# joyecnu/STTODE

Measured on AMD Instinct MI355X. Metric: predicted-trajectories/sec (20-sample best-of-K), higher is better.
Workload: dtype f32

## Files before the change

sttode_amd/csrc/chain32.hip:

```cpp
#include "chain.hpp"
#include "latency_bodies.hpp"
#include "frontend_body.hpp"
#include "api_util.hpp"
#include "../../include/sttode_hip.h"
#include <cstdlib>
#include <cstddef>

#ifdef C32_DIAG_TRACE
__shared__ long long g_tr_ph[4];
#define C32_TRACE_BEGIN() long long _tr_t0 = 0, _tr_c0 = 0; if (threadIdx.x == 0 && A.dbg) { _tr_t0 = __builtin_amdgcn_s_memrealtime(); _tr_c0 = __builtin_amdgcn_s_memtime(); }
#define C32_TRACE_END(kind) do { if (threadIdx.x == 0 && A.dbg) { \
        const long long _t1 = __builtin_amdgcn_s_memrealtime(); unsigned _hw, _xcc; \
        asm volatile("s_getreg_b32 %0, hwreg(HW_REG_HW_ID)" : "=s"(_hw)); asm volatile("s_getreg_b32 %0, hwreg(HW_REG_XCC_ID)" : "=s"(_xcc)); \
        const unsigned long long _r = atomicAdd((unsigned long long*)A.dbg, 1ull); if ((long long)_r >= A.dbg[1]) break;  \
        long long* _p = A.dbg + 8 + _r * 12; _p[0] = A.trace_tag; _p[1] = blockIdx.x; _p[2] = (kind); _p[3] = _tr_t0; _p[4] = _t1; _p[5] = _hw; _p[6] = _xcc; \
        _p[8] = g_tr_ph[0]; _p[9] = g_tr_ph[1]; _p[10] = g_tr_ph[2]; _p[7] = __builtin_amdgcn_s_memtime() - _tr_c0; _p[11] = g_tr_ph[3]; } } while (0)
#define C32_TRACE_PHASE(i) do { if (threadIdx.x == 0) g_tr_ph[i] = __builtin_amdgcn_s_memrealtime(); } while (0)
#else
#define C32_TRACE_PHASE(i) do { } while (0)
#define C32_TRACE_BEGIN() do { } while (0)
#define C32_TRACE_END(kind) do { } while (0)
#endif

#include "role_body.hpp"
// ... 443 lines not shown
            }
            const f32x4* tc = st.cur() + (i % 3) * C32_TILE_B3;
            const f32x4* tn = (i % 3 < 2) ? tc + C32_TILE_B3 : nullptr;
            if (i > 0 && i < KT1) {
                STT_FENCE();
                split3(Bh[i - 1], Bt);
            }
            f32x16& acc = i < KT1 ? h1 : acc2[i < KT1 ? 0 : i - KT1];
            if (PRE) tile_mma_b3(acc, fr[i & 1], Bt, fr[(i + 1) & 1], tn);
            else tile_mma_b3n(acc, tc, Bt);
            if (i == KT1 - 1) {
                h1 = relu16(h1);
                split3(h1, Bt);
            }
        }
        st.end();
    }
}
template <int NO, class ST>
__device__ __forceinline__ void mlp_l3_b3(ST& st, f32x16 (&acc2)[8], const float* __restrict__ b2, const float* __restrict__ b3,
                                          f32x16 (&out)[NO], int h) {
#pragma unroll
    for (int o = 0; o < NO; ++o) out[o] = ldrows(b3 + 32 * o, h);
    Frag6 fr[2];
    B3 Bt;
#pragma unroll
    for (int i = 0; i < 8 * NO; ++i) {
        if (i % NO == 0) {
            STT_FENCE();
            const f32x16 b = ldrows(b2 + 32 * (i / NO), h);
            const f32x16 a = relu16(acc2[i / NO] + b);
            split3(a, Bt);
        }
        if (i % 3 == 0) {
            if (i > 0) st.end();
            ldfrag6(fr[i & 1], st.cur());
            st.begin();
        }
        const f32x4* tn = (i % 3 < 2 && i + 1 < 8 * NO) ? st.cur() + (i % 3 + 1) * C32_TILE_B3 : nullptr;
        tile_mma_b3(out[i % NO], fr[i & 1], Bt, fr[(i + 1) & 1], tn);
    }
    st.end();
}

__device__ __forceinline__ f32x16 b3_to_f32(const B3& b) {
    f32x16 r;
#pragma unroll
    for (int kb = 0; kb < 2; ++kb) {
        const u32x4v H = __builtin_bit_cast(u32x4v, b.p[0][kb]), M = __builtin_bit_cast(u32x4v, b.p[1][kb]), L = __builtin_bit_cast(u32x4v, b.p[2][kb]);
#pragma unroll
        for (int q = 0; q < 4; ++q) {
            r[8 * kb + 2 * q] = (bf_lo(H[q]) + bf_lo(M[q])) + bf_lo(L[q]);
            r[8 * kb + 2 * q + 1] = (bf_hi(H[q]) + bf_hi(M[q])) + bf_hi(L[q]);
        }
    }
    return r;
}
template <class ST>
__device__ __forceinline__ void gru32_steps_b3(ST& st, const float* gb, const float* cb, const f32x16& d, f32x16 (&hs)[3], int Tp, int h) {
    B3 dB, hB[3];
    split3(d, dB);
#pragma unroll
    for (int j = 0; j < 3; ++j) split3(hs[j], hB[j]);
    constexpr int T = C32_TILE_B3;
#pragma unroll 1
    for (int t = 0; t < Tp; ++t) {
        B3 eB;
        {
            f32x16 e = ldrows(cb, h);
            st.begin();
            tile_mma_b3n(e, st.cur(), dB);
            e = relu16(e);
            st.end();
            split3(e, eB);
        }
        f32x16 hn[3];
#pragma unroll
        for (int j = 0; j < 3; ++j) {
            STT_FENCE();
            f32x16 ar = ldrows(gb + 0 * 96 + 32 * j, h);
            st.begin();
            tile_mma_b3n(ar, st.cur(), eB);
            tile_mma_b3n(ar, st.cur() + T, hB[0]);
            tile_mma_b3n(ar, st.cur() + 2 * T, hB[1]);
            st.end(); st.begin();
            tile_mma_b3n(ar, st.cur(), hB[2]);
#pragma unroll
            for (int r = 0; r < 16; ++r) ar[r] = C32_SIG(ar[r]);
            STT_FENCE();
            f32x16 az = ldrows(gb + 1 * 96 + 32 * j, h);
            tile_mma_b3n(az, st.cur() + T, eB);
            tile_mma_b3n(az, st.cur() + 2 * T, hB[0]);
            st.end(); st.begin();
            tile_mma_b3n(az, st.cur(), hB[1]);
            tile_mma_b3n(az, st.cur() + T, hB[2]);
#pragma unroll
            for (int r = 0; r < 16; ++r) az[r] = C32_SIG(az[r]);
            STT_FENCE();
            f32x16 an = ldrows(gb + 3 * 96 + 32 * j, h);
            tile_mma_b3n(an, st.cur() + 2 * T, hB[0]);
            st.end(); st.begin();
            tile_mma_b3n(an, st.cur(), hB[1]);
            tile_mma_b3n(an, st.cur() + T, hB[2]);
            {
                const f32x16 bi = ldrows(gb + 2 * 96 + 32 * j, h);
#pragma unroll
                for (int r = 0; r < 16; ++r) an[r] = fmaf(ar[r], an[r], bi[r]);
            }
            STT_FENCE();
            tile_mma_b3n(an, st.cur() + 2 * T, eB);
            st.end();
            const f32x16 hp = b3_to_f32(hB[j]);
#pragma unroll
            for (int r = 0; r < 16; ++r) {
                const float ng = C32_TANH(an[r]);
                hn[j][r] = fmaf(az[r], hp[r] - ng, ng);
            }
        }
#pragma unroll
        for (int j = 0; j < 3; ++j) {
            hs[j] = hn[j];
            split3(hn[j], hB[j]);
        }
    }
}

template <bool ZS, class ST>
__device__ __forceinline__ f32x16 gru32_conv(ST& st, const float* cb, const f32x16& d, int t, int Tp, int h, bool pre) {
    f32x16 e = ldrows(cb, h);
    Frag fa, fb;
    if (ZS) {
        const int k0 = 2 * t - 2, k1 = 2 * t + 3;
        const int g0 = (k0 > 0 ? k0 : 0) >> 3, g1 = (k1 < 2 * Tp - 1 ? k1 : 2 * Tp - 1) >> 3;
        const f32x4* tc = st.cur();
#pragma unroll
        for (int g = 0; g < 4; ++g)
            if (g >= g0 && g <= g1) fa.a[g] = tc[g * 64];
        st.begin(3);
#pragma unroll
        for (int g = 0; g < 4; ++g)
            if (g >= g0 && g <= g1)
#pragma unroll
                for (int r = 0; r < 4; ++r) e = __builtin_amdgcn_mfma_f32_32x32x2f32(fa.a[g][r], d[4 * g + r], e, 0, 0, 0);
        __builtin_amdgcn_sched_barrier(0);
        if (pre) st.take_prefetched();
        else st.fetch();
    } else {
        ldfrag(fa, st.cur());
        st.begin(3);
        tile_mma2f(st, e, fa, d, fb, nullptr, pre ? 0 : 1);
        if (pre) st.take_prefetched();
    }
    e = relu16(e);
    st.end();
    return e;
}

template <bool ZS, class ST>
__device__ __forceinline__ void gru32_steps(ST& st, const float* gb, const float* cb, const f32x16& d, f32x16 (&hs)[3], int Tp, int h) {
    if (ZS) {
        const f32x16 e = gru32_conv<ZS>(st, cb, d, 0, Tp, h, false);
        Frag fa, fb;
#pragma unroll
        for (int j = 0; j < 3; ++j) {
            STT_FENCE();
            f32x16 ar = ldrows(gb + 0 * 96 + 32 * j, h);
            ldfrag(fa, st.cur()); st.begin(3);
            tile_mma2f(st, ar, fa, e, fb, nullptr);
            st.end(); ldfrag(fa, st.cur() + 1 * C32_TILE); st.begin(3);
#pragma unroll
            for (int r = 0; r < 16; ++r) ar[r] = C32_SIG(ar[r]);
            STT_FENCE();
            f32x16 az = ldrows(gb + 1 * 96 + 32 * j, h);
            tile_mma2f(st, az, fa, e, fb, nullptr, 2);
            st.end(); st.begin(3);
            st.take_prefetched();
#pragma unroll
            for (int r = 0; r < 16; ++r) az[r] = C32_SIG(az[r]);
            STT_FENCE();
            f32x16 an = ldrows(gb + 3 * 96 + 32 * j, h);
            {
                const f32x16 bi = ldrows(gb + 2 * 96 + 32 * j, h);
#pragma unroll
                for (int r = 0; r < 16; ++r) an[r] = fmaf(ar[r], an[r], bi[r]);
            }
            st.end(); ldfrag(fa, st.cur() + 2 * C32_TILE);
            if (j < 2) st.begin(3); else st.begin();
            STT_FENCE();
            tile_mma2f(st, an, fa, e, fb, nullptr, (j == 2 && 1 < Tp) ? 2 : 1);
            st.end();
#pragma unroll
            for (int r = 0; r < 16; ++r) {
                const float ng = C32_TANH(an[r]);
                hs[j][r] = fmaf(az[r], 0.f - ng, ng);
            }
        }
    }
#pragma unroll 1
    for (int t = ZS ? 1 : 0; t < Tp; ++t) {
        const f32x16 e = gru32_conv<ZS>(st, cb, d, t, Tp, h, ZS);
        Frag fa, fb;
        f32x16 hn[3];
#pragma unroll
        for (int j = 0; j < 3; ++j) {
            STT_FENCE();
            f32x16 ar = ldrows(gb + 0 * 96 + 32 * j, h);
            ldfrag(fa, st.cur()); st.begin(3);
            tile_mma2f(st, ar, fa, e, fb, st.cur() + 1 * C32_TILE);
            tile_mma2(ar, fb, hs[0], fa, st.cur() + 2 * C32_TILE);
            tile_mma2(ar, fa, hs[1], fb, nullptr);
            st.end(); ldfrag(fa, st.cur()); st.begin(3);
            tile_mma2f(st, ar, fa, hs[2], fb, st.cur() + 1 * C32_TILE);
#pragma unroll
            for (int r = 0; r < 16; ++r) ar[r] = C32_SIG(ar[r]);
            STT_FENCE();
            f32x16 az = ldrows(gb + 1 * 96 + 32 * j, h);
            tile_mma2(az, fb, e, fa, st.cur() + 2 * C32_TILE);
            tile_mma2(az, fa, hs[0], fb, nullptr);
            st.end(); ldfrag(fa, st.cur()); st.begin(3);
            tile_mma2f(st, az, fa, hs[1], fb, st.cur() + 1 * C32_TILE);
            tile_mma2(az, fb, hs[2], fa, st.cur() + 2 * C32_TILE);
#pragma unroll
            for (int r = 0; r < 16; ++r) az[r] = C32_SIG(az[r]);
            STT_FENCE();
            f32x16 an = ldrows(gb + 3 * 96 + 32 * j, h);
            tile_mma2(an, fa, hs[0], fb, nullptr);
            st.end(); ldfrag(fa, st.cur());
            if (j < 2) st.begin(3); else st.begin();
            tile_mma2f(st, an, fa, hs[1], fb, st.cur() + 1 * C32_TILE, (ZS && j == 2 && t + 1 < Tp) ? 2 : 1);
            tile_mma2(an, fb, hs[2], fa, st.cur() + 2 * C32_TILE);
            {
                const f32x16 bi = ldrows(gb + 2 * 96 + 32 * j, h);
#pragma unroll
                for (int r = 0; r < 16; ++r) an[r] = fmaf(ar[r], an[r], bi[r]);
            }
            STT_FENCE();
            tile_mma2(an, fa, e, fb, nullptr);
            st.end();
#pragma unroll
            for (int r = 0; r < 16; ++r) {
                const float ng = C32_TANH(an[r]);
                hn[j][r] = fmaf(az[r], hs[j][r] - ng, ng);
            }
        }
#pragma unroll
        for (int j = 0; j < 3; ++j) hs[j] = hn[j];
    }

}

#include "role32.hpp"

__device__ __forceinline__ int opaque(int v) { asm volatile("" : "+v"(v)); return v; }

#ifdef C32_DIAG_STAMPS
#define C32_STAMP(k) do { if (threadIdx.x == 0 && A.dbg && gi < 4) { A.dbg[((size_t)blockIdx.x * 4 + gi) * 16 + 2 * (k)] = __builtin_amdgcn_s_memtime(); \
                                                                    A.dbg[((size_t)blockIdx.x * 4 + gi) * 16 + 2 * (k) + 1] = __builtin_amdgcn_s_memrealtime(); } } while (0)
#else
#define C32_STAMP(k) do { } while (0)
#endif


__host__ __device__ __forceinline__ int xcd_group(int b, int G) {
    const int x = b & 7, i = b >> 3, q = G >> 3, r = G & 7;
    return x * q + (x < r ? x : r) + i;
}

template <int NY, int FUSE, bool B3M, bool ZS>
__global__ __launch_bounds__(256, 2) void traj_chain_kernel(ChainArgs A) {
    constexpr bool kDynCount = !B3M && ((NY == 1 && FUSE == 2 && !ZS) || (NY == 2 && FUSE == 1 && ZS));
    typedef ChainStreamT<B3M ? C32_BUF_B3 : C32_CMAX * C32_TILE, B3M, kDynCount> Stream;
    extern __shared__ __attribute__((aligned(16))) char smem[];
    f32x4* ring = reinterpret_cast<f32x4*>(smem);
    f32x4* slots = ring + 2 * Stream::kBuf;
    f32x4* zslots = slots + 4 * C32_SLOT;
    float* cst = reinterpret_cast<float*>(zslots + 4 * C32_SLOT);
    int* sq = reinterpret_cast<int*>(cst + C32Const<NY>::total);
    typedef C32Const<NY> CO;

    const int lane = threadIdx.x & 63, c = lane & 31, h = lane >> 5;
    const int wave = __builtin_amdgcn_readfirstlane(threadIdx.x >> 6);
    const f32x4* slot = slots + wave * C32_SLOT;
    const f32x4* zslot = zslots + wave * C32_SLOT;
    const unsigned slot_addr = __builtin_amdgcn_readfirstlane(lds_addr(slot));
    const unsigned zslot_addr = __builtin_amdgcn_readfirstlane(lds_addr(zslot));
    const int ngroups = (A.ncols + 127) >> 7;

    C32_TRACE_BEGIN();
    if (FUSE == 2 && (int)blockIdx.x < A.R32.nwg) {
        role32_body<ZS>(*(KRole32Args*)((const __attribute__((address_space(4))) char*)__builtin_amdgcn_kernarg_segment_ptr() + offsetof(ChainArgs, R32)),
                    blockIdx.x, smem);
        C32_TRACE_END(1);
        return;
    }
    int fb = FUSE == 0 ? (int)blockIdx.x : (int)blockIdx.x - (FUSE == 2 ? A.R32.nwg : A.R.ntiles);
    if (FUSE && A.xcd_map && fb >= 0) fb = xcd_group(fb, ngroups);
    if (FUSE == 1 && fb < 0) {
        agent_role(A.R, (A.ncols + A.K - 1) / A.K, A.Tp, A.ldx, A.xpad, A.R.ntiles + fb, smem);
        C32_TRACE_END(1);
        return;
    }
    for (int i = threadIdx.x; i < CO::total; i += blockDim.x) cst[i] = A.consts[i];
    if (threadIdx.x == 0) sq[0] = FUSE == 2 ? fb : (FUSE == 0 && A.persistent) ? atomicAdd(A.counter, 1) : FUSE ? fb : (int)blockIdx.x;
    if (FUSE == 1) {
        const int g0 = fb;
        const int c_lo = g0 * 128, c_hi = (c_lo + 127 < A.ncols ? c_lo + 127 : A.ncols - 1);
        const int t_lo = (c_lo / A.K) >> 4, t_hi = (c_hi / A.K) >> 4;
        if (wave == 0) {
            const bool ok = wait_tiles(A.R.flags, t_lo, t_hi, A.R.flags + A.R.ntiles, lane, A.R.tmo_host);
            if (!ok && lane == 0) sq[0] = -1;
        }
    }
    __syncthreads();
    C32_TRACE_PHASE(3);
    int g = sq[0];
    if (FUSE == 1 && g < 0) {
        for (int i = threadIdx.x; i < 128 * A.Tf2; i += blockDim.x) {
            const size_t o = (size_t)fb * 128 * A.Tf2 + i;
            if (o < (size_t)A.ncols * A.Tf2) A.pred[o] = __builtin_nanf("");
        }
        return;
    }
    if (g >= ngroups) return;
    Stream st;
    st.init(A.pool, A.prog, A.prog_len, ring);

    auto col_of = [&](int gg) { int col = gg * 128 + wave * 32 + c; return col < A.ncols ? col : A.ncols - 1; };
    {
        const int c0 = col_of(g);
        gather_rows(A.A0x, row_off(c0 / A.K, 512, h), slot_addr);
        gather_rows(A.z, row_off(c0, 32, h), zslot_addr);
    }
    asm volatile("s_waitcnt vmcnt(0)" ::: "memory");
    __syncthreads();

    int gi = 0;
    (void)gi;
    while (true) {
        C32_STAMP(0);
        const int col = g * 128 + wave * 32 + c;
        int colc = col < A.ncols ? col : A.ncols - 1;
        int agent = colc / A.K;
        const bool live = col < A.ncols;
        __syncthreads();
        if (threadIdx.x == 0)
            sq[1] = (FUSE == 2 && A.persistent && ngroups > A.nworkers) ? A.nworkers + atomicAdd(A.counter, 1)
                    : (FUSE == 0 && A.persistent) ? atomicAdd(A.counter, 1) : ngroups;

        f32x16 acc2[8];
        f32x16 d;
        {
            agent = opaque(agent);
            f32x16 xo[1];
            const unsigned ao = row_off(agent, 512, h);
            if (B3M) {
                mlp_l12_b3<0, true>(st, slot, zslot, nullptr, A.A0x, ao, A.A0y, ao, acc2, lane);
                mlp_l3_b3<1>(st, acc2, cst + CO::b2x, cst + CO::b3x, xo, h);
            } else {
                mlp_l12<0>(st, slot, zslot, nullptr, A.A0x, ao, A.A0y, ao, acc2, lane);
                mlp_l3<1, 3>(st, acc2, cst + CO::b2x, cst + CO::b3x, xo, h);
            }
            agent = opaque(agent);
            const float* xp = A.xpad + (size_t)agent * A.ldx;
#pragma unroll
            for (int a = 0; a < 4; ++a) {
                f32x4 v = splat4(0.f);
                if (8 * a + 4 * h < A.ldx) v = ld4(xp + 8 * a + 4 * h);
#pragma unroll
                for (int b = 0; b < 4; ++b) d[4 * a + b] = v[b] - xo[0][4 * a + b];
            }
        }
        STT_FENCE();
        C32_STAMP(1);
        {
            agent = opaque(agent);
            f32x16 yo[NY];
            const unsigned ao = row_off(agent, 512, h);
            if (B3M) {
                mlp_l12_b3<0, true>(st, slot, zslot, nullptr, A.A0y, ao, A.A1y, ao, acc2, lane);
                mlp_l3_b3<NY>(st, acc2, cst + CO::b2y, cst + CO::b3y, yo, h);
            } else {
                mlp_l12<0>(st, slot, zslot, nullptr, A.A0y, ao, A.A1y, ao, acc2, lane);
                mlp_l3<NY, 1>(st, acc2, cst + CO::b2y, cst + CO::b3y, yo, h);
            }
            if (live) {
                float* prow = A.park + (size_t)opaque(col) * A.Tf2;
#pragma unroll
                for (int o = 0; o < NY; ++o)
#pragma unroll
                    for (int a = 0; a < 4; ++a) {
                        const int row0 = 32 * o + 8 * a + 4 * h;
                        float* p = prow + row0;
                        if (row0 + 3 < A.Tf2 && (A.Tf2 & 3) == 0) {
                            f32x4 v = {yo[o][4 * a], yo[o][4 * a + 1], yo[o][4 * a + 2], yo[o][4 * a + 3]};
                            st4(p, v);
                        } else {
#pragma unroll
                            for (int b = 0; b < 4; ++b)
                                if (row0 + b < A.Tf2) p[b] = yo[o][4 * a + b];
                        }
                    }
            }
        }
        STT_FENCE();
        C32_STAMP(2);
        f32x16 hs[3];
        {
#pragma unroll
            for (int j = 0; j < 3; ++j) hs[j] = splat16(0.f);
            if (B3M) gru32_steps_b3(st, cst + CO::gb, cst + CO::cb, d, hs, A.Tp, h);
            else gru32_steps<ZS>(st, cst + CO::gb, cst + CO::cb, d, hs, A.Tp, h);
        }
        STT_FENCE();
        C32_STAMP(3);
        const int gnext = sq[1];
        {
            agent = opaque(agent);
            const int cnx = col_of(gnext < ngroups ? gnext : g);
            const unsigned ao = row_off(agent, 512, h), an = row_off(cnx / A.K, 512, h);
            if (B3M) mlp_l12_b3<3, false>(st, slot, zslot, hs, A.A1y, ao, A.A0x, an, acc2, lane);
            else mlp_l12<3>(st, slot, zslot, hs, A.A1y, ao, A.A0x, an, acc2, lane);
            gather_rows(A.z, row_off(opaque(cnx), 32, h), zslot_addr);
            f32x16 yo[NY];
            if (B3M) mlp_l3_b3<NY>(st, acc2, cst + CO::b2m, cst + CO::b3m, yo, h);
            else mlp_l3<NY, 3>(st, acc2, cst + CO::b2m, cst + CO::b3m, yo, h);
            {
                agent = opaque(agent);
                const float cx = A.cur[2 * agent], cy = A.cur[2 * agent + 1];
                const float ox = A.orig[2 * agent], oy = A.orig[2 * agent + 1];
                const bool vec = (A.Tf2 & 3) == 0;
                const float* yrow = A.park + (size_t)opaque(colc) * A.Tf2;
                float* prow = A.pred + (size_t)opaque(col) * A.Tf2;
                const float* grow = FUSE == 2 && A.m_gt ? A.m_gt + (size_t)agent * A.Tf2 : nullptr;
                float dd[NY][4][2];
#pragma unroll
                for (int o = 0; o < NY; ++o)
#pragma unroll
                    for (int a = 0; a < 4; ++a) {
                        const int row0 = 32 * o + 8 * a + 4 * h;
                        const bool whole = vec && row0 + 3 < A.Tf2;
                        f32x4 y0 = splat4(0.f);
                        if (whole) y0 = ld4(yrow + row0);
                        else {
#pragma unroll
                            for (int b = 0; b < 4; ++b)
                                if (row0 + b < A.Tf2) y0[b] = yrow[row0 + b];
                        }
                        f32x4 v;
                        v[0] = ((y0[0] + yo[o][4 * a + 0]) + cx) + ox;
                        v[1] = ((y0[1] + yo[o][4 * a + 1]) + cy) + oy;
                        v[2] = ((y0[2] + yo[o][4 * a + 2]) + cx) + ox;
                        v[3] = ((y0[3] + yo[o][4 * a + 3]) + cy) + oy;
                        if (live) {
                            if (whole) st4(prow + row0, v);
                            else {
#pragma unroll
                                for (int b = 0; b < 4; ++b)
                                    if (row0 + b < A.Tf2) prow[row0 + b] = v[b];
                            }
                        }
                        dd[o][a][0] = dd[o][a][1] = 0.f;
                        if (FUSE == 2 && grow) {
                            if (row0 < A.Tf2) { const float2 g = *reinterpret_cast<const float2*>(grow + row0); dd[o][a][0] = bok_dist(v[0], v[1], g.x, g.y, A.m_scale); }
                            if (row0 + 2 < A.Tf2) { const float2 g = *reinterpret_cast<const float2*>(grow + row0 + 2); dd[o][a][1] = bok_dist(v[2], v[3], g.x, g.y, A.m_scale); }
                        }
                    }
                if (FUSE == 2 && grow) {
                    const int Tf = A.Tf2 >> 1;
                    float acc = 0.f, fdl = -1.f;
#pragma unroll
                    for (int o = 0; o < NY; ++o)
#pragma unroll
                        for (int a = 0; a < 4; ++a) {
                            const int t0 = (32 * o + 8 * a + 4 * h) >> 1;
                            float mine = acc;
                            if (h == 0) { if (t0 < Tf) mine += dd[o][a][0]; if (t0 + 1 < Tf) mine += dd[o][a][1]; }
                            float mine1 = __shfl(mine, c, 64);
                            if (h == 1) { if (t0 < Tf) mine1 += dd[o][a][0]; if (t0 + 1 < Tf) mine1 += dd[o][a][1]; }
                            acc = __shfl(mine1, c + 32, 64);
                            if (t0 == Tf - 1) fdl = dd[o][a][0];
                            if (t0 + 1 == Tf - 1) fdl = dd[o][a][1];
                        }
                    fdl = fmaxf(fdl, __shfl_xor(fdl, 32, 64));
                    const float adev = acc / (float)Tf;
                    if (live && h == 0) {
                        atomicMin(reinterpret_cast<unsigned*>(A.m_ade) + agent, __float_as_uint(adev));
                        atomicMin(reinterpret_cast<unsigned*>(A.m_fde) + agent, __float_as_uint(fdl));
                    }
                }
            }
        }
        C32_STAMP(4);
#ifdef C32_DIAG_STAMPS
        if (threadIdx.x == 0 && A.dbg && gi < 4) {
            long long* o = A.dbg + ((size_t)blockIdx.x * 4 + gi) * 16 + 10;
            o[0] = st.gap_cyc; o[1] = st.gap_n; o[2] = st.gap_cal;
        }
        st.gap_cyc = 0; st.gap_n = 0;
#endif
        ++gi;
        g = gnext;
        if (g >= ngroups) break;
    }
    C32_TRACE_END(0);
}

struct Gru32Args {
    const float* xin; int ldx;
    const f32x4* pool; const int2* prog; int prog_len;
    const float* consts;
    float* state;
    int ncols, Tp;
};
template <bool ZS>
__global__ __launch_bounds__(256, 2) void gru32_kernel(Gru32Args A) {
    extern __shared__ __attribute__((aligned(16))) char smem[];
    f32x4* ring = reinterpret_cast<f32x4*>(smem);
    float* cst = reinterpret_cast<float*>(ring + C32_RING);
    const int lane = threadIdx.x & 63, c = lane & 31, h = lane >> 5;
    const int wave = __builtin_amdgcn_readfirstlane(threadIdx.x >> 6);
    for (int i = threadIdx.x; i < 416; i += blockDim.x) cst[i] = A.consts[i];
    __syncthreads();
    ChainStream st;
    st.init(A.pool, A.prog, A.prog_len, ring);
    const int col = blockIdx.x * 128 + wave * 32 + c;
    const int colc = col < A.ncols ? col : A.ncols - 1;
    f32x16 d;
    {
        const float* xp = A.xin + (size_t)colc * A.ldx;
#pragma unroll
        for (int a = 0; a < 4; ++a) {
            f32x4 v = splat4(0.f);
            if (8 * a + 4 * h < A.ldx) v = ld4(xp + 8 * a + 4 * h);
#pragma unroll
            for (int b = 0; b < 4; ++b) d[4 * a + b] = v[b];
        }
    }
    asm volatile("s_waitcnt vmcnt(0)" ::: "memory");
    __syncthreads();
    f32x16 hs[3];
#pragma unroll
    for (int j = 0; j < 3; ++j) hs[j] = splat16(0.f);
    gru32_steps<ZS>(st, cst, cst + 384, d, hs, A.Tp, h);
    if (col < A.ncols) {
#pragma unroll
        for (int j = 0; j < 3; ++j)
#pragma unroll
            for (int a = 0; a < 4; ++a) {
                const f32x4 v = {hs[j][4 * a], hs[j][4 * a + 1], hs[j][4 * a + 2], hs[j][4 * a + 3]};
                st4(A.state + (size_t)col * 96 + 32 * j + 8 * a + 4 * h, v);
            }
    }
}

static int chain_cus() {
    static int n = 0;
    if (!n) {
        int dev = 0;
        hipDeviceProp_t p;
        if (hipGetDevice(&dev) == hipSuccess && hipGetDeviceProperties(&p, dev) == hipSuccess) n = p.multiProcessorCount;
        if (n <= 0) n = 256;
    }
    return n;
}
static int gru_zero_skip() {
    static const int v = getenv("STTODE_GRU_ZERO_SKIP") ? atoi(getenv("STTODE_GRU_ZERO_SKIP")) != 0 : 1;
    return v;
}
static int chain_lds(int NY, bool b3 = false) { return ((b3 ? 2 * C32_BUF_B3 : C32_RING) + 8 * C32_SLOT) * 16 + (1216 + 64 * NY) * 4 + 16; }

static int role_lds(int Tp) {
    const int e = (Tp * 256 + 512) * 16, g = (2 * 6 * 64 + 2 * 24 * 64 + 2 * 4 * 64) * 16;
    return e > g ? e : g;
}

static int role32_lds() { return C32_RING * 16 + R32C::total * 4; }

template <int NY, int FUSE, bool B3M = false> static int chain_launch(ChainArgs a, int wgs_per_cu, hipStream_t s) {
    void (*kern)(ChainArgs) = gru_zero_skip() ? traj_chain_kernel<NY, FUSE, B3M, true> : traj_chain_kernel<NY, FUSE, B3M, false>;
    STT_SET_LDS_ONCE(kern, 96 * 1024);
    const int ngroups = (a.ncols + 127) / 128;
    int grid = ngroups;
    if (FUSE == 1) grid = a.R.ntiles + ngroups;
    else if (FUSE == 2) {
        int workers = ngroups;
        if (a.persistent && workers > 2 * chain_cus()) workers = 2 * chain_cus();
        grid = a.R32.nwg + (a.ncols > 0 ? workers : 0);
        a.nworkers = workers;
        if (workers < ngroups) a.xcd_map = 0;
    }
    int lds = chain_lds(NY, B3M);
    if (FUSE == 1 && lds < role_lds(a.Tp)) lds = role_lds(a.Tp);
    if (FUSE == 2 && a.R32.nwg > 0 && lds < role32_lds()) lds = role32_lds();
    if (wgs_per_cu == 1 && lds < 84 * 1024) lds = 84 * 1024;
    STT_REQUIRE(lds <= 96 * 1024, "sttode_traj_chain: dynamic LDS beyond the 96 KiB the kernel is registered for");
    STT_REQUIRE((long)a.ncols * 128 <= 0xffffffffL && (long)((a.ncols + a.K - 1) / a.K) * 2048 <= 0xffffffffL,
                "sttode_traj_chain: z / per-agent table rows beyond the 32-bit byte offsets of the gathers");
    if (FUSE == 1) STT_HIP(hipMemsetAsync(a.R.flags, 0, (((size_t)a.R.ntiles + 1) * 4 + 15) / 16 * 16, s));
    hipLaunchKernelGGL(kern, dim3(grid), dim3(256), lds, s, a);
    STT_HIP(hipGetLastError());
    return 0;
}

extern "C" int sttode_gru_cols32(const float* xin, int ldx, const float* pool, const int* prog, int prog_len, const float* consts,
                                 float* state, int ncols, int Tp, void* stream) {
    STT_REQUIRE(xin && pool && prog && consts && state, "sttode_gru_cols32: null pointer");
    STT_REQUIRE(ncols > 0 && Tp >= 1 && (ldx == 16 || ldx == 32) && 2 * Tp <= ldx, "sttode_gru_cols32: bad ncols/Tp/ldx");
    STT_REQUIRE(prog_len == 13 * Tp, "sttode_gru_cols32: chunk program must hold 13 entries per step");
    Gru32Args a;
    a.xin = xin; a.ldx = ldx; a.pool = (const f32x4*)pool; a.prog = (const int2*)prog; a.prog_len = prog_len; a.consts = consts;
    a.state = state; a.ncols = ncols; a.Tp = Tp;
    const int lds = C32_RING * 16 + 416 * 4;
    hipLaunchKernelGGL(gru_zero_skip() ? gru32_kernel<true> : gru32_kernel<false>, dim3((ncols + 127) / 128), dim3(256), lds, (hipStream_t)stream, a);
    STT_HIP(hipGetLastError());
    return 0;
}

__global__ __launch_bounds__(256, 2) void sampler_qnet32_kernel(QNet32Args Q) {
    extern __shared__ __attribute__((aligned(16))) char smem[];
    f32x4* ring = reinterpret_cast<f32x4*>(smem);
    const int lane = threadIdx.x & 63, c = lane & 31, h = lane >> 5;
    const int wave = __builtin_amdgcn_readfirstlane(threadIdx.x >> 6);
    ChainStream st;
    st.init(Q.pool, Q.prog, Q.prog_len, ring);
    const int col = blockIdx.x * 128 + wave * 32 + c;
    const bool live = col < Q.n;
    const int colc = live ? col : Q.n - 1;
    f32x16 P[4];
#pragma unroll
    for (int kt = 0; kt < 4; ++kt) P[kt] = ldrows(Q.pf + (size_t)colc * 128 + 32 * kt, h);
    asm volatile("s_waitcnt vmcnt(0)" ::: "memory");
    __syncthreads();
    TileFeed<ChainStream> fd(st);
    fd.open();
    qnet32(fd, Q, P, col, colc, live, h);
    fd.close();
}

static long sampler_tiles(const SttodeSamplerPlan* p) {
    const long h1t = p->h1 / 32, h2t = p->h2 / 32;
    return 8 + h1t * (2 + h2t) + (long)p->K * h2t * (p->eps_mode ? 2 : 1);
}
const char* stt_sampler_plan_check(const SttodeSamplerPlan* p, int K) {
    if (!p || !p->pool || !p->prog || !p->biases) return "sampler plan: null pool / program / biases";
    if (p->nz != 32) return "sampler plan: nz must be 32 (one MFMA tile of rows per sample)";
    if (p->K <= 0 || (K > 0 && p->K != K)) return "sampler plan: K must be positive and equal the model's sample_k";
    if (p->h1 <= 0 || p->h1 % 32 || p->h2 <= 0 || p->h2 % 32 || p->h2 > 256) return "sampler plan: hidden widths must be multiples of 32, h2 <= 256";
    if (p->eps_mode < 0 || p->eps_mode > 2 || (p->eps_mode != 0 && !p->eps)) return "sampler plan: eps_mode 0 (mean) | 1 (shared [nz]) | 2 (per agent [n][nz]); eps required unless 0";
    if (p->prog_len <= 0 || p->prog_len > 4096) return "sampler plan: prog_len must be in [1, 4096]";
    if (3L * p->prog_len < sampler_tiles(p)) return "sampler plan: chunk program too short for the widths (<= 3 tiles per chunk)";
    return nullptr;
}
int stt_sampler_qnet(const SttodeSamplerPlan* p, const float* pf, int n, float* z, void* stream) {
    QNet32Args q;
    q.pool = (const f32x4*)p->pool; q.prog = (const int2*)p->prog; q.prog_len = p->prog_len; q.bias = p->biases;
    q.pf = pf; q.z = z; q.eps = p->eps; q.n = n; q.K = p->K; q.h1t = p->h1 / 32; q.h2t = p->h2 / 32; q.eps_mode = p->eps_mode;
    const int lds = C32_RING * 16;
    hipLaunchKernelGGL(sampler_qnet32_kernel, dim3((n + 127) / 128), dim3(256), lds, (hipStream_t)stream, q);
    STT_HIP(hipGetLastError());
    return 0;
}
extern "C" int sttode_sampler_qnet(const SttodeSamplerPlan* plan, const float* pf, int n, float* z, void* stream) {
    STT_REQUIRE(plan && pf && z, "sttode_sampler_qnet: null pointer");
    STT_REQUIRE(n > 0 && (long)n * plan->K <= 0x7fffffffL / 32, "sttode_sampler_qnet: n must be positive (and n K 32 within int range)");
    if (const char* why = stt_sampler_plan_check(plan, 0)) {
        char b[256];
        snprintf(b, sizeof(b), "sttode_sampler_qnet: %s", why);
        stt_set_error(b);
        return 1;
    }
    return stt_sampler_qnet(plan, pf, n, z, stream);
}

#if defined(C32_DIAG_STAMPS) || defined(C32_DIAG_TRACE)
static long long* g_chain_dbg = nullptr;
static int g_trace_tag = 0;
extern "C" int sttode_chain_debug_buffer(void* p) { g_chain_dbg = (long long*)p; return 0; }
#endif

extern "C" int sttode_chain_prog_len(int Tp, int Tf) {
    const int NY = (2 * Tf + 31) / 32;
    const int l3y = (8 * NY + 2) / 3;
    return (48 + 3) + (48 + l3y) + 13 * Tp + (64 + l3y);
}

static int traj_chain_impl(const float* A0x, const float* A0y, const float* A1y, const float* pool, const int* prog, int prog_len,
                           const float* consts, const float* z, const float* xpad, int ldx, const float* cur, const float* orig,
                           float* pred, int* counter, int ncols, int K, int Tp, int Tf, int wgs_per_cu, bool b3, void* stream) {
    STT_REQUIRE(A0x && A0y && A1y && pool && prog && consts && z && xpad && cur && orig && pred && counter, "sttode_traj_chain: null pointer");
    STT_REQUIRE(ncols > 0 && K > 0 && Tp >= 1 && 2 * Tp <= 32 && Tf >= 1, "sttode_traj_chain: bad ncols/K/Tp/Tf");
    STT_REQUIRE(ldx == 16 || ldx == 32, "sttode_traj_chain: ldx must be 16 or 32");
    STT_REQUIRE(wgs_per_cu == 1 || wgs_per_cu == 2, "sttode_traj_chain: wgs_per_cu must be 1 or 2");
    STT_REQUIRE(2 * Tp <= ldx, "sttode_traj_chain: xpad rows shorter than 2*Tp");
    STT_REQUIRE(prog_len == sttode_chain_prog_len(Tp, Tf), "sttode_traj_chain: chunk program length does not match (Tp, Tf)");
    ChainArgs a;
    a.A0x = A0x; a.A0y = A0y; a.A1y = A1y; a.pool = (const f32x4*)pool; a.prog = (const int2*)prog; a.prog_len = prog_len;
    a.consts = consts; a.z = z; a.xpad = xpad; a.ldx = ldx; a.cur = cur; a.orig = orig; a.pred = pred; a.park = pred; a.counter = counter;
    a.ncols = ncols; a.K = K; a.Tp = Tp; a.Tf2 = 2 * Tf;
    a.dbg = nullptr; a.trace_tag = 0; a.xcd_map = 0; a.nworkers = 0; a.m_gt = nullptr; a.m_ade = a.m_fde = nullptr; a.m_scale = 1.0f;
    a.R = RoleArgs();
    a.persistent = 0;
#if defined(C32_DIAG_STAMPS) || defined(C32_DIAG_TRACE)
    a.dbg = g_chain_dbg;
    a.trace_tag = g_trace_tag++;
#endif
    const int NY = (2 * Tf + 31) / 32;
    hipStream_t s = (hipStream_t)stream;
    if (b3) {
        switch (NY) {
            case 1: return chain_launch<1, 0, true>(a, wgs_per_cu, s);
            case 2: return chain_launch<2, 0, true>(a, wgs_per_cu, s);
            case 3: return chain_launch<3, 0, true>(a, wgs_per_cu, s);
            default: STT_REQUIRE(false, "sttode_traj_chain: future length beyond the built instantiations (2*Tf <= 96)");
        }
    }
    switch (NY) {
        case 1: return chain_launch<1, 0>(a, wgs_per_cu, s);
        case 2: return chain_launch<2, 0>(a, wgs_per_cu, s);
        case 3: return chain_launch<3, 0>(a, wgs_per_cu, s);
        default: STT_REQUIRE(false, "sttode_traj_chain: future length beyond the built instantiations (2*Tf <= 96)");
    }
    return 0;
}
extern "C" int sttode_traj_chain(const float* A0x, const float* A0y, const float* A1y, const float* pool, const int* prog, int prog_len,
                                 const float* consts, const float* z, const float* xpad, int ldx, const float* cur, const float* orig,
                                 float* pred, int* counter, int ncols, int K, int Tp, int Tf, int wgs_per_cu, void* stream) {
    return traj_chain_impl(A0x, A0y, A1y, pool, prog, prog_len, consts, z, xpad, ldx, cur, orig, pred, counter, ncols, K, Tp, Tf, wgs_per_cu, false, stream);
}
int stt_traj_chain_b3(const float* A0x, const float* A0y, const float* A1y, const float* pool, const int* prog, int prog_len,
                      const float* consts, const float* z, const float* xpad, int ldx, const float* cur, const float* orig,
                      float* pred, int* counter, int ncols, int K, int Tp, int Tf, int wgs_per_cu, void* stream) {
    return traj_chain_impl(A0x, A0y, A1y, pool, prog, prog_len, consts, z, xpad, ldx, cur, orig, pred, counter, ncols, K, Tp, Tf, wgs_per_cu, true, stream);
}

bool stt_chain_fused_covers(int Tp) { return Tp >= 2 && 2 * Tp <= 32 && role_lds(Tp) <= 80 * 1024; }
int stt_chain_fused(const float* const* W, float* ws, const long* off, int n, int K, int Tp, int Tf, int prog_len, const float* z, float* pred,
                    float ode_time, const float* attn, int ld_attn, int wgs_per_cu, int b3, int drop_tile, unsigned* tmo_host, void* stream) {
    STT_REQUIRE(W && ws && off && z && pred, "stt_chain_fused: null pointer");
    STT_REQUIRE(n > 0 && K > 0 && stt_chain_fused_covers(Tp) && Tf >= 1, "stt_chain_fused: shape outside the fused launch");
    STT_REQUIRE(!attn || (ld_attn >= 64 && ld_attn % 4 == 0), "stt_chain_fused: bad attention leading dimension");
    STT_REQUIRE(prog_len == sttode_chain_prog_len(Tp, Tf), "stt_chain_fused: chunk program length does not match (Tp, Tf)");
    STT_REQUIRE((long)n * K <= 0x7fffffffL, "stt_chain_fused: too many trajectories");
    ChainArgs a;
    a.A0x = ws + off[STT_B_A0X]; a.A0y = ws + off[STT_B_A0Y]; a.A1y = ws + off[STT_B_A1Y];
    a.pool = (const f32x4*)W[b3 ? STT_W_CHAINB3_POOL : STT_W_CHAIN_POOL]; a.prog = (const int2*)W[b3 ? STT_W_CHAINB3_PROG : STT_W_CHAIN_PROG];
    a.prog_len = prog_len;
    a.consts = W[STT_W_CHAIN_CONSTS]; a.z = z; a.xpad = ws + off[STT_B_XPAD]; a.ldx = 2 * Tp <= 16 ? 16 : 32; a.cur = ws + off[STT_B_CUR];
    a.orig = ws + off[STT_B_ORIG]; a.pred = pred; a.park = pred; a.counter = (int*)(ws + off[STT_B_QUEUE]);
    a.ncols = n * K; a.K = K; a.Tp = Tp; a.Tf2 = 2 * Tf; a.persistent = 0; a.dbg = nullptr; a.trace_tag = 0; a.xcd_map = 0; a.nworkers = 0;
    a.m_gt = nullptr; a.m_ade = a.m_fde = nullptr; a.m_scale = 1.0f;
#if defined(C32_DIAG_STAMPS) || defined(C32_DIAG_TRACE)
    a.dbg = g_chain_dbg;
    a.trace_tag = g_trace_tag++;
#endif
    RoleArgs& r = a.R;
    role_args_fill(r, W, ws, off);
    r.attn = attn; r.ld_attn = ld_attn;
    r.past = nullptr; r.scene_ptr = nullptr; r.S = 0;
    r.flags = (unsigned*)(ws + off[STT_B_FLAGS]); r.ntiles = (n + 15) / 16; r.ode_time = ode_time;
    r.tmo_host = tmo_host;
    a.xcd_map = 1;
    r.drop_tile = drop_tile;
    const int NY = (2 * Tf + 31) / 32;
    hipStream_t s = (hipStream_t)stream;
    switch (NY) {
        case 1: return b3 ? chain_launch<1, 1, true>(a, wgs_per_cu, s) : chain_launch<1, 1>(a, wgs_per_cu, s);
        case 2: return b3 ? chain_launch<2, 1, true>(a, wgs_per_cu, s) : chain_launch<2, 1>(a, wgs_per_cu, s);
        case 3: return b3 ? chain_launch<3, 1, true>(a, wgs_per_cu, s) : chain_launch<3, 1>(a, wgs_per_cu, s);
        default: STT_REQUIRE(false, "stt_chain_fused: future length beyond the built instantiations (2*Tf <= 96)");
    }
    return 0;
}

bool stt_chain_lagged_covers(int Tp) { return Tp >= 2 && 2 * Tp <= 32; }
int stt_chain_lagged(const float* const* W, const LagRoles& lr, const LagGroups& lg, int K, int Tp, int Tf, int prog_len, int b3, void* stream) {
    float* ws_r = lr.ws; const long* off_r = lr.off; const int n_r = lr.n; const float* attn = lr.attn; const int ld_attn = lr.ld_attn;
    const float ode_time = lr.ode_time; float* zgen = lr.zgen; const unsigned long long zkey = lr.zkey; const float* past = lr.past;
    const int* scene_ptr = lr.scene_ptr; const int S = lr.S; float* r_ade = lr.ade; float* r_fde = lr.fde;
    float* ws_g = lg.ws; const long* off_g = lg.off; const int n_g = lg.n; const float* z = lg.z; float* pred = lg.pred;
    const float* g_gt = lg.gt; float* g_ade = lg.ade; float* g_fde = lg.fde; const float g_scale = lg.scale; const int lag_workers_ok = lg.workers;
    STT_REQUIRE(W && (ws_r || ws_g), "stt_chain_lagged: nothing to launch");
    STT_REQUIRE(K > 0 && stt_chain_lagged_covers(Tp) && Tf >= 1, "stt_chain_lagged: shape outside the lagged launch");
    ChainArgs a;
    a.R = RoleArgs();
    a.R32 = Role32Args();
    a.dbg = nullptr; a.trace_tag = 0; a.xcd_map = 0; a.persistent = 0; a.counter = nullptr; a.nworkers = 0;
    a.K = K; a.Tp = Tp; a.Tf2 = 2 * Tf; a.ldx = 2 * Tp <= 16 ? 16 : 32; a.ncols = 0;
    a.pool = (const f32x4*)W[b3 ? STT_W_CHAINB3_POOL : STT_W_CHAIN_POOL]; a.prog = (const int2*)W[b3 ? STT_W_CHAINB3_PROG : STT_W_CHAIN_PROG];
    a.prog_len = prog_len; a.consts = W[STT_W_CHAIN_CONSTS];
    a.A0x = a.A0y = a.A1y = nullptr; a.z = nullptr; a.xpad = nullptr; a.cur = a.orig = nullptr; a.pred = nullptr; a.park = nullptr;
    a.m_gt = nullptr; a.m_ade = a.m_fde = nullptr; a.m_scale = 1.0f;
    if (ws_g && g_gt) {
        STT_REQUIRE(g_ade && g_fde, "stt_chain_lagged: fused metrics need ade and fde");
        a.m_gt = g_gt; a.m_ade = g_ade; a.m_fde = g_fde; a.m_scale = g_scale;
    }
    if (ws_g) {
        STT_REQUIRE(off_g && z && pred && n_g > 0 && (long)n_g * K <= 0x7fffffffL, "stt_chain_lagged: bad group arguments");
        STT_REQUIRE(prog_len == sttode_chain_prog_len(Tp, Tf), "stt_chain_lagged: chunk program length does not match (Tp, Tf)");
        a.A0x = ws_g + off_g[STT_B_A0X]; a.A0y = ws_g + off_g[STT_B_A0Y]; a.A1y = ws_g + off_g[STT_B_A1Y];
        a.z = z; a.xpad = ws_g + off_g[STT_B_XPAD]; a.cur = ws_g + off_g[STT_B_CUR]; a.orig = ws_g + off_g[STT_B_ORIG]; a.pred = pred;
        a.park = ws_g + off_g[STT_B_YBUF];
        a.ncols = n_g * K;
        a.persistent = lag_workers_ok ? 1 : 0;
        a.counter = (int*)(ws_g + off_g[STT_B_QUEUE]);
        a.xcd_map = 1;
    }
    if (ws_r) {
        STT_REQUIRE(off_r && n_r > 0, "stt_chain_lagged: bad role arguments");
        STT_REQUIRE(!attn || (ld_attn >= 64 && ld_attn % 4 == 0), "stt_chain_lagged: bad attention leading dimension");
        Role32Args& r = a.R32;
        r.pool = (const f32x4*)W[STT_W_ROLE32_POOL];
        r.prog = (const int2*)W[attn ? STT_W_ROLE32_PROG_NBA : STT_W_ROLE32_PROG_SCENES];
        r.consts = W[attn ? STT_W_ROLE32_CONSTS_NBA : STT_W_ROLE32_CONSTS_SCENES];
        r.kte = (4 * Tp + 31) / 32;
        const int e = attn ? 8 : 2 * r.kte + 8;
        r.prog_len = attn ? 13 * Tp + (e + 2) / 3 + (128 + 288 + 2) / 3 : 13 * Tp + (e + 128 + 288 + 2) / 3;
        r.enc_in = ws_r + off_r[STT_B_ENC_IN]; r.last = (const int*)(ws_r + off_r[STT_B_LAST]);
        r.g_in = ws_r + off_r[STT_B_G]; r.attn = attn; r.ld_attn = ld_attn;
        r.xpad = ws_r + off_r[STT_B_XPAD]; r.ldx = a.ldx;
        r.pf = ws_r + off_r[STT_B_PF]; r.state0 = ws_r + off_r[STT_B_STATE0];
        r.A0x = ws_r + off_r[STT_B_A0X]; r.A0y = ws_r + off_r[STT_B_A0Y]; r.A1y = ws_r + off_r[STT_B_A1Y];
        r.n = n_r; r.Tp = Tp; r.nwg = (n_r + 127) / 128; r.ode_time = ode_time;
        r.prio = 3;
        r.counter = (int*)(ws_r + off_r[STT_B_QUEUE]);
        r.zgen = zgen; r.zkey0 = (unsigned)zkey; r.zkey1 = (unsigned)(zkey >> 32); r.K = K;
        STT_REQUIRE(!past || (scene_ptr && S > 0 && !attn), "stt_chain_lagged: the in-role front-end needs scene_ptr, S > 0 and attention length 1");
        r.past = past; r.scene_ptr = scene_ptr; r.S = S;
        r.scene_orig = ws_r + off_r[STT_B_SCENE_ORIG]; r.agent_scene = (int*)(ws_r + off_r[STT_B_AGENT_SCENE]);
        r.enc_in_w = ws_r + off_r[STT_B_ENC_IN]; r.xpad_w = ws_r + off_r[STT_B_XPAD]; r.cur_w = ws_r + off_r[STT_B_CUR];
        r.orig_w = ws_r + off_r[STT_B_ORIG]; r.last_w = (int*)(ws_r + off_r[STT_B_LAST]);
        r.m_ade = r_ade; r.m_fde = r_fde;
    }
#if defined(C32_DIAG_STAMPS) || defined(C32_DIAG_TRACE)
    a.dbg = g_chain_dbg;
    a.trace_tag = g_trace_tag++;
#endif
    const int NY = (2 * Tf + 31) / 32;
    hipStream_t s = (hipStream_t)stream;
    switch (NY) {
        case 1: return b3 ? chain_launch<1, 2, true>(a, 2, s) : chain_launch<1, 2>(a, 2, s);
        case 2: return b3 ? chain_launch<2, 2, true>(a, 2, s) : chain_launch<2, 2>(a, 2, s);
        case 3: return b3 ? chain_launch<3, 2, true>(a, 2, s) : chain_launch<3, 2>(a, 2, s);
        default: STT_REQUIRE(false, "stt_chain_lagged: future length beyond the built instantiations (2*Tf <= 96)");
    }
    return 0;
}
```

sttode_amd/csrc/role_body.hpp:

```cpp
#pragma once
#include "latency_bodies.hpp"
#include "frontend_body.hpp"
#include "../../include/sttode_hip.h"

#ifndef C32_TRACE_PHASE
#define C32_TRACE_PHASE(i) do { } while (0)
#endif

struct RoleArgs {
    EmbedW ew; PostW pw;
    const float* enc_in; const int* last; float* g; float* qkv; float* pf;
    const f32x4* convP; const float* convB; const f32x4* wihP; const f32x4* whhP; const float* gbias; float* state0;
    const f32x4* WAx; const float* b1x; const f32x4* WAy; const float* b1y; const f32x4* WA1; const float* b11;
    float* A0x; float* A0y; float* A1y;
    const float* past; const int* scene_ptr; int S; float* scene_orig; int* agent_scene;
    float* enc_in_w; float* xpad_w; float* cur_w; float* orig_w; int* last_w;
    const float* attn; int ld_attn;
    unsigned* flags;
    unsigned* tmo_host;
    int ntiles; float ode_time;
    int drop_tile;
};

#ifndef ROLE_PRIO
#define ROLE_PRIO 3
#endif

__device__ __forceinline__ void role_frontend(const RoleArgs& R, int nag, int Tp, int ldx, int tile, bool enc, bool traj) {
    if (threadIdx.x < 16) {
        const int a = tile * 16 + (int)threadIdx.x;
        if (a < nag) {
            int lo = 0, hi = R.S - 1;
            while (lo < hi) {
                const int mid = (lo + hi + 1) >> 1;
                if (R.scene_ptr[mid] <= a) lo = mid; else hi = mid - 1;
            }
            const int a0 = R.scene_ptr[lo], a1 = R.scene_ptr[lo + 1];
            float sx = 0.f, sy = 0.f;
            for (int aa = a0; aa < a1; ++aa) {
                sx += R.past[((size_t)aa * Tp + (Tp - 1)) * 2 + 0];
                sy += R.past[((size_t)aa * Tp + (Tp - 1)) * 2 + 1];
            }
            const float inv = (float)(a1 - a0);
            const float ox = sx / inv, oy = sy / inv;
            if (enc) {
                if (a == a0) { R.scene_orig[2 * lo] = ox; R.scene_orig[2 * lo + 1] = oy; }
                R.agent_scene[a] = lo;
            }
            agent_inputs_core<true, 16>(a, R.past, Tp, ldx / 16, 1, ox, oy, a == a1 - 1, nullptr, traj ? R.xpad_w : nullptr, enc ? R.enc_in_w : nullptr,
                                    traj ? R.cur_w : nullptr, traj ? R.orig_w : nullptr, enc ? R.last_w : nullptr);
        }
    }
}

__device__ __forceinline__ void agent_role(const RoleArgs& R, int nag, int Tp, int ldx, const float* __restrict__ xpad, int tile, char* smem) {
    __builtin_amdgcn_s_setprio(ROLE_PRIO);
    if (R.attn == nullptr) {
        embed_lat_body(R.ew, R.enc_in, R.last, R.g, R.qkv, nag, Tp, tile, reinterpret_cast<f32x4*>(smem));
        __syncthreads();
    }
    C32_TRACE_PHASE(0);
    post_attn_body<false>(R.pw, R.g, R.attn ? R.attn : R.qkv + 128, R.attn ? R.ld_attn : 192, R.pf, nag, R.ode_time, 0, 1, nullptr, nullptr, tile,
                          reinterpret_cast<f32x4(*)[4][64]>(smem));
    __syncthreads();
    C32_TRACE_PHASE(1);
    f32x4 (*sH)[6][64] = reinterpret_cast<f32x4(*)[6][64]>(smem);
    f32x4* sW45 = reinterpret_cast<f32x4*>(smem) + 2 * 6 * 64;
    const int cur = ldx == 16 ? gru_lat4_body<1>(xpad, R.convP, R.convB, R.wihP, R.whhP, R.gbias, R.state0, nag, Tp, tile, sH, sW45)
                                : gru_lat4_body<2>(xpad, R.convP, R.convB, R.wihP, R.whhP, R.gbias, R.state0, nag, Tp, tile, sH, sW45);
    C32_TRACE_PHASE(2);
    const int lane = threadIdx.x & 63, c = lane & 15, q = lane >> 4;
    const int wv = __builtin_amdgcn_readfirstlane(threadIdx.x >> 6);
    const int col = tile * 16 + c;
    const int colc = col < nag ? col : nag - 1;
    f32x4 B[14];
#pragma unroll
    for (int T = 0; T < 8; ++T) B[T] = ld4(R.pf + (size_t)colc * 128 + 16 * T + 4 * q);
#pragma unroll
    for (int T = 0; T < 6; ++T) B[8 + T] = sH[cur][T][lane];
    preact_rows<14, true>(R.WAx, R.b1x, R.A0x, B, col, col < nag, lane, q, wv);
    preact_rows<14, true>(R.WAy, R.b1y, R.A0y, B, col, col < nag, lane, q, wv);
    preact_rows<8, true>(R.WA1, R.b11, R.A1y, B, col, col < nag, lane, q, wv);
    asm volatile("s_waitcnt vmcnt(0)" ::: "memory");
    __syncthreads();
    if (threadIdx.x == 0 && tile != R.drop_tile) __hip_atomic_store(R.flags + tile, 1u, __ATOMIC_RELAXED, __HIP_MEMORY_SCOPE_AGENT);
}

__device__ __forceinline__ bool wait_tiles(unsigned* flags, int t_lo, int t_hi, unsigned* tmo, int lane, unsigned* tmo_host = nullptr) {
    bool ok = true;
    for (int t = t_lo + lane; t <= t_hi; t += 64) {
        unsigned spins = 0;
        while (true) {
            const unsigned v = __hip_atomic_load(flags + t, __ATOMIC_RELAXED, __HIP_MEMORY_SCOPE_AGENT);
            if (v != 0u) break;
            __builtin_amdgcn_s_sleep(32);
            if (++spins > (1u << 20)) { ok = false; break; }
        }
    }
    ok = __all(ok);
    if (!ok && lane == 0) {
        __hip_atomic_store(tmo, 1u, __ATOMIC_RELAXED, __HIP_MEMORY_SCOPE_AGENT);
        if (tmo_host) __hip_atomic_store(tmo_host, 1u, __ATOMIC_RELAXED, __HIP_MEMORY_SCOPE_SYSTEM);
    }
    __builtin_amdgcn_fence(__ATOMIC_ACQUIRE, "agent");
    asm volatile("s_waitcnt vmcnt(0)" ::: "memory");
    return ok;
}

__device__ __forceinline__ void role_publish(unsigned* flag, bool really, unsigned val = 1u) {
    asm volatile("s_waitcnt vmcnt(0)" ::: "memory");
    __syncthreads();
    if (threadIdx.x == 0 && really) __hip_atomic_store(flag, val, __ATOMIC_RELAXED, __HIP_MEMORY_SCOPE_AGENT);
}

static inline void role_args_fill(RoleArgs& r, const float* const* W, float* ws, const long* off) {
    r.tmo_host = nullptr;
    r.ew.fc1P = W[STT_W_FC1P]; r.ew.fc1b = W[STT_W_FC1B]; r.ew.posP = (const f32x4*)W[STT_W_POSP]; r.ew.peb = W[STT_W_PEB];
    r.ew.fc2P = (const f32x4*)W[STT_W_FC2P]; r.ew.fc2b = W[STT_W_FC2B]; r.ew.fc3P = (const f32x4*)W[STT_W_FC3P]; r.ew.fc3b = W[STT_W_FC3B];
    r.ew.fc3last = W[STT_W_FC3LAST]; r.ew.inP = (const f32x4*)W[STT_W_INP]; r.ew.inb = W[STT_W_INB];
    r.pw.outP = (const f32x4*)W[STT_W_OUTP]; r.pw.outb = W[STT_W_OUTB]; r.pw.infoP = (const f32x4*)W[STT_W_INFOP]; r.pw.infob = W[STT_W_INFOB];
    r.pw.gateP = (const f32x4*)W[STT_W_GATEP]; r.pw.gateb = W[STT_W_GATEB]; r.pw.ln1w = W[STT_W_LN1W]; r.pw.ln1b = W[STT_W_LN1B];
    r.pw.l1P = (const f32x4*)W[STT_W_L1P]; r.pw.l1b = W[STT_W_L1B]; r.pw.l2P = (const f32x4*)W[STT_W_L2P]; r.pw.l2b = W[STT_W_L2B];
    r.pw.ln2w = W[STT_W_LN2W]; r.pw.ln2b = W[STT_W_LN2B];
    r.enc_in = ws + off[STT_B_ENC_IN]; r.last = (const int*)(ws + off[STT_B_LAST]); r.g = ws + off[STT_B_G]; r.qkv = ws + off[STT_B_QKV];
    r.pf = ws + off[STT_B_PF];
    r.convP = (const f32x4*)W[STT_W_B0_CONVP]; r.convB = W[STT_W_B0_CONVB]; r.wihP = (const f32x4*)W[STT_W_B0_WIHP];
    r.whhP = (const f32x4*)W[STT_W_B0_WHHP]; r.gbias = W[STT_W_B0_GBIAS]; r.state0 = ws + off[STT_B_STATE0];
    r.WAx = (const f32x4*)W[STT_W_B0_XWA]; r.b1x = W[STT_W_B0_XB1]; r.WAy = (const f32x4*)W[STT_W_B0_YWA]; r.b1y = W[STT_W_B0_YB1];
    r.WA1 = (const f32x4*)W[STT_W_B1_YWA]; r.b11 = W[STT_W_B1_YB1];
    r.A0x = ws + off[STT_B_A0X]; r.A0y = ws + off[STT_B_A0Y]; r.A1y = ws + off[STT_B_A1Y];
    r.scene_orig = ws + off[STT_B_SCENE_ORIG]; r.agent_scene = (int*)(ws + off[STT_B_AGENT_SCENE]);
    r.enc_in_w = ws + off[STT_B_ENC_IN]; r.xpad_w = ws + off[STT_B_XPAD]; r.cur_w = ws + off[STT_B_CUR]; r.orig_w = ws + off[STT_B_ORIG];
    r.last_w = (int*)(ws + off[STT_B_LAST]);
}
```

Measured before the change: 87.06 million.

## Cap fused producer-consumer chain workers and hand out column groups via tickets

In the FUSE==1 path, the grid no longer launches one consumer workgroup per column group. It launches at most 2×CUs persistent workers (overridable by env var), which claim further groups through an atomic ticket counter stored after the tile flags. Each claim waits on the producer tile flags and writes NaN poison on timeout. This is meant to cut launch and residency pressure from many waiting consumer workgroups spinning on flags, and to let producers get CUs. The cost is serialized per-group claims and dependence on a counter that must be zeroed by the enlarged memset.

Measured after the change: 87.03 million. No clear change (-0.0%).

```diff
diff --git a/sttode_amd/csrc/chain32.hip b/sttode_amd/csrc/chain32.hip
--- a/sttode_amd/csrc/chain32.hip
+++ b/sttode_amd/csrc/chain32.hip
@@ -769,25 +769,35 @@
     }
     for (int i = threadIdx.x; i < CO::total; i += blockDim.x) cst[i] = A.consts[i];
     if (threadIdx.x == 0) sq[0] = FUSE == 2 ? fb : (FUSE == 0 && A.persistent) ? atomicAdd(A.counter, 1) : FUSE ? fb : (int)blockIdx.x;
-    if (FUSE == 1) {
-        const int g0 = fb;
-        const int c_lo = g0 * 128, c_hi = (c_lo + 127 < A.ncols ? c_lo + 127 : A.ncols - 1);
-        const int t_lo = (c_lo / A.K) >> 4, t_hi = (c_hi / A.K) >> 4;
-        if (wave == 0) {
-            const bool ok = wait_tiles(A.R.flags, t_lo, t_hi, A.R.flags + A.R.ntiles, lane, A.R.tmo_host);
-            if (!ok && lane == 0) sq[0] = -1;
-        }
+    const bool tickets = FUSE == 1 && ngroups > A.nworkers;
+    auto claim = [&](int cand) {
+        bool gave_up = sq[2] != 0;
+        while (cand < ngroups) {
+            const int c_lo = cand * 128, c_hi = (c_lo + 127 < A.ncols ? c_lo + 127 : A.ncols - 1);
+            const int t_lo = (c_lo / A.K) >> 4, t_hi = (c_hi / A.K) >> 4;
+            const int ln = opaque((int)threadIdx.x) & 63;
+            if (wait_tiles(A.R.flags, t_lo, t_hi, A.R.flags + A.R.ntiles, ln, A.R.tmo_host, gave_up ? 0u : 1u << 20)) break;
+            gave_up = true;
+            sq[2] = opaque(1);
+            const float poison = __int_as_float(opaque(0x7fc00000));
+            for (int i = ln; i < 128 * A.Tf2; i += 64) {
+                const size_t o = (size_t)cand * 128 * A.Tf2 + i;
+                if (o < (size_t)A.ncols * A.Tf2) A.pred[o] = poison;
+            }
+            int t = 0;
+            if (tickets && ln == 0) t = atomicAdd(A.counter, 1);
+            cand = tickets ? A.nworkers + __builtin_amdgcn_readfirstlane(t) : ngroups;
+        }
+        return cand;
+    };
+    if (FUSE == 1 && wave == 0) {
+        sq[2] = 0;
+        const int g0 = claim(fb);
+        if (lane == 0) sq[0] = g0;
     }
     __syncthreads();
     C32_TRACE_PHASE(3);
     int g = sq[0];
-    if (FUSE == 1 && g < 0) {
-        for (int i = threadIdx.x; i < 128 * A.Tf2; i += blockDim.x) {
-            const size_t o = (size_t)fb * 128 * A.Tf2 + i;
-            if (o < (size_t)A.ncols * A.Tf2) A.pred[o] = __builtin_nanf("");
-        }
-        return;
-    }
     if (g >= ngroups) return;
     Stream st;
     st.init(A.pool, A.prog, A.prog_len, ring);
@@ -810,7 +820,17 @@
         int agent = colc / A.K;
         const bool live = col < A.ncols;
         __syncthreads();
-        if (threadIdx.x == 0)
+        if (FUSE == 1) {
+            if (wave == 0) {
+                int nx = ngroups;
+                if (tickets) {
+                    int t = 0;
+                    if (threadIdx.x == 0) t = atomicAdd(A.counter, 1);
+                    nx = claim(A.nworkers + __builtin_amdgcn_readfirstlane(t));
+                }
+                if (threadIdx.x == 0) sq[1] = nx;
+            }
+        } else if (threadIdx.x == 0)
             sq[1] = (FUSE == 2 && A.persistent && ngroups > A.nworkers) ? A.nworkers + atomicAdd(A.counter, 1)
                     : (FUSE == 0 && A.persistent) ? atomicAdd(A.counter, 1) : ngroups;
 
@@ -1034,6 +1054,10 @@
     static const int v = getenv("STTODE_GRU_ZERO_SKIP") ? atoi(getenv("STTODE_GRU_ZERO_SKIP")) != 0 : 1;
     return v;
 }
+static int fused_workers() {
+    static const int v = getenv("STTODE_FUSED_WORKERS") ? atoi(getenv("STTODE_FUSED_WORKERS")) : -1;
+    return v;
+}
 static int chain_lds(int NY, bool b3 = false) { return ((b3 ? 2 * C32_BUF_B3 : C32_RING) + 8 * C32_SLOT) * 16 + (1216 + 64 * NY) * 4 + 16; }
 
 static int role_lds(int Tp) {
@@ -1048,8 +1072,14 @@
     STT_SET_LDS_ONCE(kern, 96 * 1024);
     const int ngroups = (a.ncols + 127) / 128;
     int grid = ngroups;
-    if (FUSE == 1) grid = a.R.ntiles + ngroups;
-    else if (FUSE == 2) {
+    if (FUSE == 1) {
+        const int cap = fused_workers() < 0 ? 2 * chain_cus() : fused_workers();
+        const int workers = cap > 0 && ngroups > cap ? cap : ngroups;
+        grid = a.R.ntiles + workers;
+        a.nworkers = workers;
+        a.counter = (int*)(a.R.flags + a.R.ntiles + 1);
+        if (workers < ngroups) a.xcd_map = 0;
+    } else if (FUSE == 2) {
         int workers = ngroups;
         if (a.persistent && workers > 2 * chain_cus()) workers = 2 * chain_cus();
         grid = a.R32.nwg + (a.ncols > 0 ? workers : 0);
@@ -1063,7 +1093,7 @@
     STT_REQUIRE(lds <= 96 * 1024, "sttode_traj_chain: dynamic LDS beyond the 96 KiB the kernel is registered for");
     STT_REQUIRE((long)a.ncols * 128 <= 0xffffffffL && (long)((a.ncols + a.K - 1) / a.K) * 2048 <= 0xffffffffL,
                 "sttode_traj_chain: z / per-agent table rows beyond the 32-bit byte offsets of the gathers");
-    if (FUSE == 1) STT_HIP(hipMemsetAsync(a.R.flags, 0, (((size_t)a.R.ntiles + 1) * 4 + 15) / 16 * 16, s));
+    if (FUSE == 1) STT_HIP(hipMemsetAsync(a.R.flags, 0, (((size_t)a.R.ntiles + 2) * 4 + 15) / 16 * 16, s));
     hipLaunchKernelGGL(kern, dim3(grid), dim3(256), lds, s, a);
     STT_HIP(hipGetLastError());
     return 0;
diff --git a/sttode_amd/csrc/role_body.hpp b/sttode_amd/csrc/role_body.hpp
--- a/sttode_amd/csrc/role_body.hpp
+++ b/sttode_amd/csrc/role_body.hpp
@@ -86,7 +86,8 @@
     if (threadIdx.x == 0 && tile != R.drop_tile) __hip_atomic_store(R.flags + tile, 1u, __ATOMIC_RELAXED, __HIP_MEMORY_SCOPE_AGENT);
 }
 
-__device__ __forceinline__ bool wait_tiles(unsigned* flags, int t_lo, int t_hi, unsigned* tmo, int lane, unsigned* tmo_host = nullptr) {
+__device__ __forceinline__ bool wait_tiles(unsigned* flags, int t_lo, int t_hi, unsigned* tmo, int lane, unsigned* tmo_host = nullptr,
+                                           unsigned bound = 1u << 20) {
     bool ok = true;
     for (int t = t_lo + lane; t <= t_hi; t += 64) {
         unsigned spins = 0;
@@ -94,7 +95,7 @@
             const unsigned v = __hip_atomic_load(flags + t, __ATOMIC_RELAXED, __HIP_MEMORY_SCOPE_AGENT);
             if (v != 0u) break;
             __builtin_amdgcn_s_sleep(32);
-            if (++spins > (1u << 20)) { ok = false; break; }
+            if (++spins > bound) { ok = false; break; }
         }
     }
     ok = __all(ok);
```
